# eflynn8/pharmacophore-diffusion

Hardware: AMD Instinct MI355X
Metric: denoising steps/sec (batch x T) at 256-atom pocket, 6 centers (higher is better)
Workload: dtype f32; 1 GPU; BASELINE config 2: 256-atom pocket, 6 centers, T=500 schedule, batch=32 per GPU, dev.yml network; batch_per_gpu=32, n_prot=256, n_pharm=6, T=500, parallelism=graphs sharded over 1 GPU(s), no data-path collective

## Files before the change

include/pfdyn.h:

```cpp
#ifndef PFDYN_H
#define PFDYN_H

#include <stdint.h>

#ifdef __cplusplus
extern "C" {
#endif

#define PF_ABI_VERSION 1

typedef struct pf_handle pf_handle;
typedef void* pf_stream;

typedef enum pf_status {
    PF_OK = 0,
    PF_ERR_ARG = -1,
    PF_ERR_HIP = -2,
    PF_ERR_STATE = -3,
    PF_ERR_WEIGHT = -4,
    PF_ERR_EXCHANGE = -5
} pf_status;

#define PF_NORM_MEAN 0
#define PF_NORM_VALUE 1
// ... 112 lines not shown
                        pf_stream stream);
#define PF_NUM_KERNEL_CLASSES 9
int pf_profile_enable(pf_handle* h, uint32_t kernel_mask);
int pf_profile_read(pf_handle* h, double* total_ms , int64_t* launches , pf_stream stream);
int pf_profile_read_train(pf_handle* h, double* total_ms , int64_t* launches , pf_stream stream);
int pf_debug_work(pf_handle* h, double* flops, double* bytes, int64_t* n_edges , double* executed_flops,
                  int64_t* executed_edges , pf_stream stream);
int pf_debug_counts(pf_handle* h, int64_t* out , pf_stream stream);
int pf_debug_kernel_family(pf_handle* h, int32_t layer, int32_t* rows_per_wave);
int pf_debug_ahead(pf_handle* h, int64_t* out , pf_stream stream);
int pf_debug_pa_check(pf_handle* h, int64_t* violations , pf_stream stream);
int pf_debug_xchg_timeouts(pf_handle* h, int32_t* n);
int pf_debug_xchg_fault(pf_handle* h, int32_t drop_word, int32_t poll_max);
int pf_debug_last_eps(pf_handle* h, float* dev_eps_h , float* dev_eps_x , pf_stream stream);
int pf_debug_l0_hoist(pf_handle* h, int32_t* rows_per_wave);
int pf_debug_chain(pf_handle* h, int32_t kind, int32_t layer, int32_t sub, int32_t n_rows, const float* dev_s_in,
                   const float* dev_v_in, float* dev_s_out, float* dev_v_out, pf_stream stream);

#ifdef __cplusplus
}
#endif
#endif
```

pharmacophore-diffusion_amd/_lib.py:

```python
import ctypes
import os

_HERE = os.path.dirname(os.path.abspath(__file__))
LIB_PATH = os.environ.get("PFDYN_LIB") or os.path.join(_HERE, "csrc", "libpfdyn.so")

PF_ABI_VERSION = 1
PF_NORM_MEAN, PF_NORM_VALUE, PF_NORM_GRAPH = 0, 1, 2


class PfConfig(ctypes.Structure):
    _fields_ = [
        ("abi_version", ctypes.c_int32), ("pharm_nf", ctypes.c_int32), ("rec_nf", ctypes.c_int32),
        ("vector_size", ctypes.c_int32), ("n_hidden_scalars", ctypes.c_int32), ("n_convs", ctypes.c_int32),
        ("n_message_gvps", ctypes.c_int32), ("n_update_gvps", ctypes.c_int32), ("n_noise_gvps", ctypes.c_int32),
        ("message_norm_mode", ctypes.c_int32), ("message_norm_value", ctypes.c_float),
        ("ff_k", ctypes.c_int32), ("pf_k", ctypes.c_int32),
        ("cutoff_pp", ctypes.c_float), ("cutoff_pf", ctypes.c_float), ("cutoff_fp", ctypes.c_float),
        ("cutoff_ff", ctypes.c_float), ("rbf_dmax", ctypes.c_float), ("rbf_dim", ctypes.c_int32),
    ]


class PfStepCoef(ctypes.Structure):
    _fields_ = [("t", ctypes.c_float), ("alpha_t_given_s", ctypes.c_float), ("var_terms", ctypes.c_float),
                ("sigma", ctypes.c_float), ("ep_zt", ctypes.c_float), ("ep_pred", ctypes.c_float)]
# ... 40 lines not shown
    "pf_debug_get_edges": (_I64, [_P, _I32, _P, _P, _I64, _P]),
    "pf_debug_conv_layer": (ctypes.c_int, [_P, _I32] + [_P] * 11),
    "pf_profile_enable": (ctypes.c_int, [_P, ctypes.c_uint32]),
    "pf_profile_read": (ctypes.c_int, [_P, ctypes.POINTER(ctypes.c_double), ctypes.POINTER(_I64), _P]),
    "pf_profile_read_train": (ctypes.c_int, [_P, ctypes.POINTER(ctypes.c_double), ctypes.POINTER(_I64), _P]),
    "pf_debug_work": (ctypes.c_int, [_P, ctypes.POINTER(ctypes.c_double), ctypes.POINTER(ctypes.c_double),
                                     ctypes.POINTER(_I64), ctypes.POINTER(ctypes.c_double), ctypes.POINTER(_I64), _P]),
    "pf_debug_counts": (ctypes.c_int, [_P, ctypes.POINTER(_I64), _P]),
    "pf_debug_kernel_family": (ctypes.c_int, [_P, ctypes.c_int32, ctypes.POINTER(ctypes.c_int32)]),
    "pf_debug_last_eps": (ctypes.c_int, [_P, _P, _P, _P]),
    "pf_debug_xchg_timeouts": (ctypes.c_int, [_P, ctypes.POINTER(ctypes.c_int32)]),
    "pf_debug_xchg_fault": (ctypes.c_int, [_P, _I32, _I32]),
    "pf_debug_ahead": (ctypes.c_int, [_P, ctypes.POINTER(_I64), _P]),
    "pf_debug_pa_check": (ctypes.c_int, [_P, ctypes.POINTER(_I64), _P]),
    "pf_debug_l0_hoist": (ctypes.c_int, [_P, ctypes.POINTER(ctypes.c_int32)]),
    "pf_debug_chain": (ctypes.c_int, [_P, _I32, _I32, _I32, _I32, _P, _P, _P, _P, _P]),
}

_lib = None


def load():
    global _lib
    if _lib is not None:
        return _lib
    if not os.path.exists(LIB_PATH):
        raise ImportError(
            f"{LIB_PATH} is missing: the HIP extension has not been built "
            "(run `python -c 'import __graft_entry__ as g; g.build()'` or `make -C pharmacophore-diffusion_amd/csrc`). "
            "There is no CPU fallback.")
# ... 19 lines not shown
```

pharmacophore-diffusion_amd/csrc/pf_device.h:

```cpp
#pragma once
#include <stdint.h>

#define PF_S 128
#define PF_V 16
#define PF_R 16
#define PF_MAXF 64
#define PF_MAXK 16
#define PF_MAX_GVPS 8

enum { ET_FF = 0, ET_PF = 1, ET_FP = 2, ET_PP = 3 };

#if defined(__HIP_DEVICE_COMPILE__)
#define PF_AS1 __attribute__((address_space(1)))
#else
#define PF_AS1
#endif
typedef const float PF_AS1* pf_gcf;

struct GvpW {
    pf_gcf a_wh;
    pf_gcf a_wu;
    pf_gcf a_main;
    pf_gcf a_main_c;
    pf_gcf a_gate_c;
// ... 123 lines not shown
    const int* ptype;
    const int* eorig;
    const int* l0_gid;
    const float* l0c;
    int ngroups_sel;
    const int* need; int need_stamp;
    int pa_abs;
    pf_gcf n16[4]; int n16_stride[4];
    int uni_base[3], uni_s01, uni_s2g, uni_pa_groups;
    int ptab16_off[4];
    const float* pcen; int pcen_nf;
    const float* x0_static;
    const int* pa_skip;
    int* cnt_snap;
    int* pa_gstamp; int pa_serial;
};

#define L0H_WR 0
#define L0H_WSH 2048
#define L0H_B 4224
#define L0H_WH0 4352
#define L0H_WU 4384
#define L0H_BG 4672
#define L0H_WHT 4736
#define L0H_WHT_PF 21120
#define L0H_B_PF 37504
#define L0H_SIZE (37504 + 128)
#define L0C_WHT_FF 0
#define L0C_B_FF 16384
#define L0C_WHT_FP 16512
#define L0C_B_FP 32896
// ... 253 lines not shown
```

pharmacophore-diffusion_amd/csrc/pf_host.cpp:

```cpp
#include <hip/hip_runtime.h>

#include <algorithm>
#include <cmath>
#include <cstdio>
#include <cstdlib>
#include <cstring>
#include <ctime>
#include <map>
#include <string>
#include <unordered_map>
#include <climits>
#include <vector>

#include "../../include/pfdyn.h"
#include "pf_device.h"
#include "pf_train.h"

#define L0_PTAB_SLOTS 2048

extern "C" {
void pfk_edge_msg(const EdgeParams* p, int layer0, hipStream_t s);
void pfk_edge_msg_coop(const EdgeParams* p, int layer0, hipStream_t s);
void pfk_edge_msg_coop2(const EdgeParams* p, int layer0, hipStream_t s);
void pfk_node_update_coop(const NodeParams* p, int layer0, hipStream_t s);
// ... 80 lines not shown

static void linspace_f32(float start, float end, int steps, float* out) {
    const float step = (end - start) / (float)(steps - 1);
    const int half = steps / 2;
    for (int i = 0; i < steps; ++i) out[i] = i < half ? start + step * (float)i : end - step * (float)(steps - i - 1);
}

}

struct LaunchPolicy {
    static constexpr int kCUs = 256, kSIMDs = 4 * kCUs;
    int n16_mask = 7;
    int tail_graphs_max = 256;
    int xcd_split = 1;
    int edge_rec = 1;
    int node_static = 1;
    int node_xcds = 2;
    int fused_uni = 1;
    int xchg_sleep = 1, hsb_avoid = 0;
    int hs_build = 1;
    int tail_form = 4;
    long n16_fuse_rows_max = 20000;
    long n16_rows_max = 24000;
    int rg_rows_max = 1 << 30;
    int rg2_rows_min = 12000;
    int rg2_rows_min_node = 12000;
    int rg2p_rows_min = 11000;
    int rg2_rows_min_hoist = 30000;
    int l0_rga = 0, l0_rgp = 0;
    int rg_split_max = 128;
// ... 11 lines not shown
        geti("PFDYN_COOP_EDGE_MAX", coop_edge_max); geti("PFDYN_COOP_NODE_MAX", coop_node_max);
        if (const char* e = getenv("PFDYN_COOP2_EDGE_MAX")) coop2_edge_max = coop2_dense_max = atoi(e);
        if (const char* e = getenv("PFDYN_RG_SPLIT_MAX")) rg_split_max = rg_split_max_node = rg_split_max_head = atoi(e);
        geti("PFDYN_RG_SPLIT_MAX_NODE", rg_split_max_node); geti("PFDYN_RG_SPLIT_MAX_HEAD", rg_split_max_head);
        geti("PFDYN_RG_ROWS_MAX", rg_rows_max);
        if (const char* e = getenv("PFDYN_RG2_ROWS_MIN")) rg2_rows_min = rg2_rows_min_hoist = rg2p_rows_min = rg2_rows_min_node = atoi(e);
        geti("PFDYN_RG2P_ROWS_MIN", rg2p_rows_min); geti("PFDYN_RG2_ROWS_MIN_NODE", rg2_rows_min_node); geti("PFDYN_RG2_ROWS_MIN_HOIST", rg2_rows_min_hoist);
        geti("PFDYN_L0_RGP", l0_rgp); geti("PFDYN_L0_RGA", l0_rga);
        for (const char* v : {"PFDYN_RG2_ROWS_MIN", "PFDYN_RG2P_ROWS_MIN", "PFDYN_RG2_ROWS_MIN_HOIST", "PFDYN_RG_SPLIT_MAX", "PFDYN_L0_RGA",
                              "PFDYN_L0_RGP", "PFDYN_RG_ROWS_MAX"})
            if (getenv(v)) n16_mask = 0;
        geti("PFDYN_N16", n16_mask);
        geti("PFDYN_TAIL_GRAPHS_MAX", tail_graphs_max);
        geti("PFDYN_XCD_SPLIT", xcd_split);
        geti("PFDYN_EDGE_REC", edge_rec);
        geti("PFDYN_NODE_XCDS", node_xcds); geti("PFDYN_NODE_STATIC", node_static); geti("PFDYN_HS_BUILD", hs_build); geti("PFDYN_FUSED_UNI", fused_uni); geti("PFDYN_XCHG_SLEEP", xchg_sleep); geti("PFDYN_HSB_AVOID", hsb_avoid);
        if (const char* e = getenv("PFDYN_TAIL_FORM")) tail_form = (e[0] == 'n' || atoi(e) == 16) ? 16 : 4;
        if (const char* e = getenv("PFDYN_N16_ROWS_MAX")) n16_rows_max = n16_fuse_rows_max = atol(e);
        if (const char* e = getenv("PFDYN_N16_FUSE_ROWS_MAX")) n16_fuse_rows_max = atol(e);
    }
};

struct pf_handle {
    LaunchPolicy pol;
    pf_config cfg{};
    bool spec = true, wide = false;
    std::vector<size_t> wide_off;
    WideGvp* d_wgvp = nullptr;
    size_t wide_out_w = 0, wide_out_b = 0;
    std::string err;
// ... 78 lines not shown
    int xchg_fault = 0, xchg_poll_max = 0;
    size_t n16_l0h[4] = {0, 0, 0, 0}, n16_l0h_stride[4] = {0, 0, 0, 0};
    size_t l0c_off = 0;
    bool cen_hoist = true;
    float *d_cen_h = nullptr, *d_cen_p = nullptr, *d_snap[2] = {nullptr, nullptr};
    unsigned int* d_xchg2 = nullptr;
    int snap_cur = -1;
    std::vector<float> t_plan; size_t plan_pos = 0;
    bool cen_valid = false; float cen_t = 0.f; uint64_t cen_wver = 0;
    bool last_cen = false;
    bool pa_spec = true;
    bool spec_valid = false; float spec_t = 0.f; uint64_t spec_wver = 0;
    int step_id = 2;
    int *d_pa_stamp = nullptr, *d_pa_same = nullptr;
    bool e0_saved = false; EdgeParams e0{}; EncodeParams ep0{}; int e0_groups = 0;
    int last_spec = 0;
    int* d_pa_cnt = nullptr;
    int pa_spec_split = 0;
    bool pa_check = false;
    int pa_serial = 0, spec_serial = 0;
    int* d_pa_gstamp = nullptr;
    unsigned long long* d_pa_chk = nullptr;
    bool no_fixed_shapes = false;
    ScaleArgs pend_scale{}; bool has_pend_scale = false;
    bool no_fix_fuse = false;
    bool train_bf16 = false;
    bool train_node_save = true;
    std::vector<float*> t_nsv_z, t_nsv_g, t_nsv_v;
    std::vector<char> t_node_saved;
    std::vector<int> t_grp;
// ... 748 lines not shown
        lp.nt = m; lp.t_dev = nullptr; lp.ptab = h->d_ptab + (size_t)slot0 * slot_floats;
        pfk_l0_hoist(&lp, 1, s);
    }
}

static void n16_refresh(pf_handle* h, hipStream_t s) {
    if (!h->n16_stale) return;
    pfk_gather_weights(h->d_flat, h->d_map + h->n16_begin, h->n_packed - h->n16_begin, h->d_w + h->n16_begin, s);
    if (h->n_split_tab) pfk_n16_split_words(h->d_flat, h->d_split_tab, h->n_split_tab, h->d_w, s);
    h->n16_stale = false;
}

static int run_dynamics_wide(pf_handle* h, float* eps_h, float* eps_x, hipStream_t s, const float* t_scalar) {
    const pf_config& c = h->cfg;
    h->tail_done = false; h->last_tail = 0; h->last_hoist = 0;
    h->cen_valid = false; h->last_cen = false; h->spec_valid = false; h->last_spec = 0; h->e0_saved = false;
    if (h->share_ok && h->share_check == 0) (void)share_now(h);
    if (h->share_check == 2)
        PF_FAIL(h, PF_ERR_ARG, "pf_set_pocket_groups: the claim made for this batch is false -- a graph differs from its representative in "
                               "coordinates or features (compared on the device); bind the batch again without the claim");
    const int S = c.n_hidden_scalars, V = c.vector_size;
    WideEncParams ep{};
    ep.Np = h->Np; ep.Nf = h->Nf; ep.S = S; ep.rec_nf = c.rec_nf; ep.pharm_nf = c.pharm_nf;
    ep.prot_h0 = h->d_prot_h0; ep.pharm_h = h->d_pharm_h;
    ep.t = t_scalar ? nullptr : h->d_t; ep.t_scalar = t_scalar ? *t_scalar : 0.f; ep.gid = h->d_gid;
    for (int nt = 0; nt < 2; ++nt) {
        ep.w[nt] = h->d_w + h->enc_w[nt]; ep.b[nt] = h->d_w + h->enc_b[nt];
        ep.ln_w[nt] = h->d_w + h->enc_lw[nt]; ep.ln_b[nt] = h->d_w + h->enc_lb[nt];
    }
    ep.h_out = h->d_h[0];
    { ProfScope ps(h, pf_handle::K_ENCODE, s); pfk_wide_encode(&ep, s); }
// ... 120 lines not shown
    }
    if (l == 0 && dc.cen_have && h->n16_l0h[ET_FF] != 0) {
        for (int et : {(int)ET_FF, (int)ET_FP}) { e.n16[et] = h->d_w + h->n16_l0h[et]; e.n16_stride[et] = (int)h->n16_l0h_stride[et]; }
        e.pcen = h->d_cen_p; e.pcen_nf = h->Nf; h->last_cen = true;
    }
    e.ngroups_sel = region_groups(h, shared, 0, e.nreg, 16);
    int stride[3], cap[3], grp[3] = {0, 0, 0};
    bool uni = l == 0 && h->pol.fused_uni && !shared && e.reg == h->d_reg && e.nreg == 4 * h->B && h->B <= 64 && !e.pa_abs && !e.need &&
               uniform_regions(h, 3, stride, cap);
    for (int et = 0; et < 3 && uni; ++et) { grp[et] = (cap[et] + 15) / 16; uni = grp[et] > 0 && grp[et] < 8; }
    if (uni) {
        for (int et = 0; et < 3; ++et) e.uni_base[et] = h->h_reg[(size_t)et * h->B];
        e.uni_s01 = stride[0] | (stride[1] << 16);
        e.uni_s2g = stride[2] | (grp[0] << 16) | (grp[1] << 19) | (grp[2] << 22) | ((h->B - 1) << 25);
        e.uni_pa_groups = region_groups(h, shared, 3 * h->B, 4 * h->B, 16);
    }
    dc.rg = 4;
    if (l == 0 && e.x0_static && pa_ahead_ok(h, e, shared)) {
        e.cnt_snap = h->d_pa_cnt;
        h->e0 = e; h->ep0 = dc.ep; h->e0_saved = true;
        h->e0_groups = region_groups(h, shared, 3 * h->B, 4 * h->B, 16);
    }
}
static void edge_launch(DynCall& dc, int l) {
    pf_handle* h = dc.h; hipStream_t s = dc.s; const pf_config& c = h->cfg; const bool train = dc.train;
    const bool last = dc.last = (l == c.n_convs - 1), pruned = dc.pruned = (l == prune_layer(h));
    EdgeParams& e = dc.e; int &rg = dc.rg, &rgp = dc.rgp;
    e = edge_params_base(h, l, last, pruned);
    e.h = train ? h->t_H[l] : h->d_h[dc.cur]; e.v = train ? h->t_V[l] : h->d_v[dc.cur];
    e.msg_s = train ? h->t_msg_s[l] : h->d_msg_s; e.msg_v = train ? h->t_msg_v[l] : h->d_msg_v;
    if (dc.fuse_l0node && l == 1) { e.msg_s = h->d_msg_s2; e.msg_v = h->d_msg_v2; }
    e.pre = (l == 0 && dc.pre_ready) ? h->d_pre : nullptr;
    if (train) { e.sv_z = h->t_sv_z[l]; e.sv_g = h->t_sv_g[l]; e.sv_v = h->t_sv_v[l]; e.sv_stride = (size_t)std::max<int64_t>(h->Ecap, 1); }
    const bool shared = dc.shared = dc.share && pruned && l == 0;
    if ((last || pruned) && h->rg_compact && (last ? 2 : 4) * h->B <= 1024) {
        e.reg = shared ? h->d_reg_share : h->d_reg; e.regB = h->B; e.nreg = (last ? 2 : 4) * h->B; e.pa_abs = shared ? 1 : 0;
        if (shared) { e.need = h->d_need; e.need_stamp = h->edges_stamp; }
        e.ngroups4 = region_groups(h, shared, 0, e.nreg, 4); e.ngroups8 = region_groups(h, shared, 0, e.nreg, 8);
    }
    if (train && h->train_bf16) e.bf16 = 1;
    rg = train ? ((h->train_rg_edge && h->train_rg_node && !h->train_bf16) ? h->pol.rg_mode(e.ntiles) : 0)
               : h->pol.rg_mode(shared ? (int)((h->share_rows + 31) / 32) : e.ntiles);
    rgp = 0;
// ... 87 lines not shown
    pf_handle* h = dc.h; const StepParams* step = dc.step;
    cp.on = 1; cp.Nf = h->Nf; cp.nf = h->cfg.pharm_nf; cp.t_next = t_next; cp.pharm_h = h->d_snap[h->snap_cur]; cp.noise = step->noise;
    cp.a_ts = step->a_ts; cp.var = step->var; cp.sigma = step->sigma; cp.ep_zt = step->ep_zt; cp.ep_pred = step->ep_pred; cp.ep_feat = step->ep_feat;
    cp.enc_w = h->d_w + h->enc_w[1]; cp.enc_b = h->d_w + h->enc_b[1]; cp.enc_lw = h->d_w + h->enc_lw[1]; cp.enc_lb = h->d_w + h->enc_lb[1];
    cp.blk = h->d_w + h->l0c_off; cp.cen_h = h->d_cen_h; cp.cen_p = h->d_cen_p; cp.xchg2 = hp.xchg2 = h->d_xchg2;
    h->cen_valid = true; h->cen_t = t_next; h->cen_wver = h->w_version;
}
static int pa_ahead_plan(DynCall& dc, EdgeParams& es, EncodeParams& ees) {
    pf_handle* h = dc.h; const pf_config& c = h->cfg;
    if (!(h->e0_saved && h->pa_spec && !h->t_plan.empty() && dc.t_scalar && h->d_pa_stamp && !share_next(h))) return 0;
    float tn = planned_next_t(h, *dc.t_scalar, nullptr);
    if (tn != tn) return 0;
    l0_prepare_t(h, &tn, 1, dc.s);
    uint32_t bits; memcpy(&bits, &tn, 4);
    es = h->e0; es.pa_skip = nullptr; es.pcen = nullptr;
    es.ptab = h->d_ptab + (size_t)h->ptab_slot[bits] * L0_NTAB * c.rec_nf * PF_S;
    for (int et = 0; et < 4; ++et) { es.n16[et] = h->d_w + h->n16_l0[et]; es.n16_stride[et] = (int)h->n16_l0_stride[et]; }
    ees = h->ep0; ees.t_scalar = tn;
    h->spec_valid = true; h->spec_t = tn; h->spec_wver = h->w_version;
    es.pa_serial = h->spec_serial = ++h->pa_serial; es.pa_gstamp = h->d_pa_gstamp;
    return h->e0_groups;
}
static void merged_step_launch(DynCall& dc, const NodeParams& n, HeadParams& hp) {
    pf_handle* h = dc.h; hipStream_t s = dc.s; const pf_config& c = h->cfg;
    hp.xchg = h->d_xchg; hp.xchg_fault = h->xchg_fault;
    CenHoistParams cp{}; EdgeParams es{}; EncodeParams ees{};
    const float t_next = cen_hoist_plan(dc);
    const int spec_groups = pa_ahead_plan(dc, es, ees);
    if (t_next == t_next) cen_hoist_params(dc, t_next, cp, hp);
    const bool sn = share_next(h);
// ... 68 lines not shown
        up.sv_z = h->t_hsv_z; up.sv_g = h->t_hsv_g; up.sv_v = h->t_hsv_v; up.sv_stride = (size_t)h->Nf;
        { ProfScope ps(h, pf_handle::K_HEAD, s); pfk_rg_unit(&up, s); }
        h->t_head_saved = true; dc.head_done = true;
    }
    if (!dc.head_done) { ProfScope ps(h, pf_handle::K_HEAD, s); if (hp.ntiles <= h->pol.coop_node_max) pfk_noise_head_coop(&hp, s); else pfk_noise_head(&hp, s); }
}
static int run_dynamics(pf_handle* h, float* eps_h, float* eps_x, hipStream_t s, const float* t_scalar = nullptr, bool train = false, const StepParams* step = nullptr) {
    if (h->wide && !train) return run_dynamics_wide(h, eps_h, eps_x, s, t_scalar);
    const pf_config& c = h->cfg;
    h->tail_done = false; h->last_tail = 0;
    DynCall dc{};
    dc.h = h; dc.s = s; dc.eps_h = eps_h; dc.eps_x = eps_x; dc.t_scalar = t_scalar; dc.train = train; dc.step = step;
    dc.cen_have = !train && h->cen_valid && h->edges_built && t_scalar != nullptr && *t_scalar == h->cen_t && h->cen_wver == h->w_version;
    h->cen_valid = false; h->last_cen = false;
    dc.spec_have = !train && h->spec_valid && h->edges_built && t_scalar != nullptr && *t_scalar == h->spec_t && h->spec_wver == h->w_version;
    h->spec_valid = false; h->last_spec = 0; h->e0_saved = false;
    if (!train) n16_refresh(h, s);
    dc.ep = encode_params(h, t_scalar, train ? h->t_H[0] : h->d_h[0]);
    if (const int rc = dyn_prologue(dc)) return rc;
    dyn_hoist_prepare(dc);
    h->last_hoist = 0;
    dc.fuse_l0node = !train && dc.n16_batch && (long)h->n_edge_tiles_act * 32 <= h->pol.n16_fuse_rows_max && (h->pol.n16_mask & 4) && (h->pol.n16_mask & 1) && dc.hoist && c.n_convs == 2 && prune_layer(h) == 0 && c.pf_k > 0 &&
                     c.n_update_gvps >= 1 && h->rg_compact && 2 * h->B <= 1024 && h->d_msg_s2 != nullptr && h->n16_fused[0] != 0;
    for (int l = 0; l < c.n_convs; ++l, dc.cur ^= 1) { edge_launch(dc, l); node_launch(dc, l); }
    head_launch(dc);
    h->edges_built = h->tail_done;
    hipError_t e = hipGetLastError();
    if (e != hipSuccess) PF_FAIL(h, PF_ERR_HIP, "kernel launch failed: %s", hipGetErrorString(e));
    return PF_OK;
}

// ... 1931 lines not shown
    else if (kind == 1) {
        if (sub > 1) PF_FAIL(h, PF_ERR_ARG, "pf_debug_chain: node type 0 (prot) or 1 (pharm)");
        p.stream = h->d_w + h->rg_upd[(size_t)layer * 2 + sub]; p.n_gvps = c.n_update_gvps;
    } else if (kind == 2) {
        const size_t* lo = &h->ln_off[(size_t)(layer * 2 + (sub >> 1)) * 4];
        p.ln_w = h->d_w + lo[(sub & 1) * 2]; p.ln_b = h->d_w + lo[(sub & 1) * 2 + 1];
    } else {
        p.stream = h->d_w + h->rg_upd[(size_t)(c.n_convs - 1) * 2 + 1]; p.n_gvps = c.n_noise_gvps; p.skip_gvps = c.n_update_gvps;
    }
    pfk_rg_unit(&p, (hipStream_t)stream);
    hipError_t e = hipGetLastError();
    if (e != hipSuccess) PF_FAIL(h, PF_ERR_HIP, "kernel launch failed: %s", hipGetErrorString(e));
    return PF_OK;
}

int pf_debug_l0_hoist(pf_handle* h, int32_t* rows_per_wave) {
    if (!h || !rows_per_wave) return PF_ERR_ARG;
    *rows_per_wave = h->last_hoist;
    return PF_OK;
}

int pf_profile_enable(pf_handle* h, uint32_t kernel_mask) {
    if (!h) return PF_ERR_ARG;
    h->prof_mask = kernel_mask;
    return PF_OK;
}

static int profile_read_range(pf_handle* h, int k0, int k1, double* total_ms, int64_t* launches, pf_stream stream) {
    if (!h || !total_ms || !launches) return PF_ERR_ARG;
    PF_HIP(h, hipStreamSynchronize((hipStream_t)stream));
// ... 84 lines not shown
```

pharmacophore-diffusion_amd/csrc/pf_n16.hip:

```cpp
#include <hip/hip_runtime.h>
#include <type_traits>
#include <algorithm>
#include "pf_device.h"
#ifdef N16_STAMPS
#define N16_STAMP_GLOBALS 1
namespace {
__device__ unsigned long long* g_n16_stamps = nullptr;
__device__ int g_n16_stamp_off = 0;
__device__ int g_n16_stamp_kid = -1;
}
#define SB_STAMP(k)                                                                                                    \
    do {                                                                                                               \
        const int rb_ = (int)blockIdx.x - g_n16_stamp_off;                                                             \
        if ((k) < 16 && (threadIdx.x & 63) == 0 && g_n16_stamps && rb_ >= 0 && rb_ < 64 && (g_n16_stamp_kid < 0 || g_n16_stamp_kid == 3)) \
            g_n16_stamps[((size_t)rb_ * 4 + (threadIdx.x >> 6)) * 64 + 40 + (k)] = __builtin_amdgcn_s_memtime();       \
    } while (0)
#endif
#include "pf_stepbuild.h"

#include "pf_n16_core.h"

using namespace pfn16;

namespace {
// ... 141 lines not shown
    const int rs = a_reg[r];
    const int ng = ((c + 15) >> 4) - keep;
    int incl = ng;
    incl += dpp_i<0x111>(incl); incl += dpp_i<0x112>(incl); incl += dpp_i<0x114>(incl); incl += dpp_i<0x118>(incl);
    incl += dpp_ir<0x142, 0xa>(incl); incl += dpp_ir<0x143, 0xc>(incl);
    const unsigned long long m = __ballot(incl > w);
    if (!m) return;
    const int l = __builtin_amdgcn_readfirstlane(__ffsll((long long)m) - 1);
    const int first = __builtin_amdgcn_readlane(incl - ng, l);
    const int cnt = __builtin_amdgcn_readlane(c, l), start = __builtin_amdgcn_readlane(rs, l);
    const int loc = (w - first + __builtin_amdgcn_readlane(keep, l)) << 4;
    const int e0 = start + loc;
    const int nv = __builtin_amdgcn_readfirstlane(min(16, cnt - loc));
    const int e = e0 + min(j, nv - 1);
    n16_edge_item<N16_M0H>(p, ep, &lds, e, a_esrc[e], a_edst[e], nv, (int)ET_PP, lane, wq, sk);
}

struct N16LnPre { float a, b; };
__device__ __forceinline__ N16LnPre n16_ln_request(pf_gcf w1, pf_gcf b1, pf_gcf w2, pf_gcf b2, const int lane, const int wq) {
    const int t = wq * 64 + lane;
    N16LnPre q;
    q.a = (t < 128 ? w1 : b1)[t & 127];
    q.b = (t < 128 ? w2 : b2)[t & 127];
    return q;
}
__device__ __forceinline__ void n16_ln_stage(const N16LnPre& q, N16Lds* lds, const int lane, const int wq) {
    const int t = wq * 64 + lane;
    lds->ln[t] = q.a;
    lds->ln[256 + t] = q.b;
}
// ... 590 lines not shown
        }
    }
}

}

extern "C" {
void pfk_n16_edge(const EdgeParams* p, const EncodeParams* enc, int layer0, hipStream_t s) {
    if (p->ntiles == 0) return;
    const int grid = p->nreg > 0 ? p->ngroups_sel : p->ntiles * 2;
    if (grid <= 0) return;
    const EncodeParams noenc{};
    if (layer0 && p->uni_s2g != 0) {
        const int B = p->regB;
        const int nstat = B * (((p->uni_s2g >> 16) & 7) + ((p->uni_s2g >> 19) & 7) + ((p->uni_s2g >> 22) & 7));
        hipLaunchKernelGGL(k_n16_edge_u, dim3(nstat + p->uni_pa_groups), dim3(256), 0, s, p->dyn_cnt, p->esrc, p->edst, p->uni_base[0],
                           p->uni_base[1], p->uni_base[2], p->uni_s01, p->uni_s2g, p->reg, *p, *enc);
        return;
    }
    if (layer0) hipLaunchKernelGGL((k_n16_edge<true>), dim3(grid), dim3(256), 0, s, p->dyn_cnt, p->reg, p->nreg, p->regB, p->pa_abs, *p, *enc);
    else hipLaunchKernelGGL((k_n16_edge<false>), dim3(grid), dim3(256), 0, s, p->dyn_cnt, p->reg, p->nreg, p->regB, p->pa_abs, *p, noenc);
}
#ifdef N16_STAMPS
int pfk_n16_set_stamp_buffer(unsigned long long* dev, int off) {
    (void)hipMemcpyToSymbol(HIP_SYMBOL(g_n16_stamp_off), &off, sizeof(off));
    return (int)hipMemcpyToSymbol(HIP_SYMBOL(g_n16_stamps), &dev, sizeof(dev));
}
int pfk_n16_set_stamp_kernel(int kid) { return (int)hipMemcpyToSymbol(HIP_SYMBOL(g_n16_stamp_kid), &kid, sizeof(kid)); }
#endif
#ifdef N16_TRACE
int pfk_n16_set_trace_buffer(unsigned long long* dev) { return (int)hipMemcpyToSymbol(HIP_SYMBOL(g_n16_trace), &dev, sizeof(dev)); }
// ... 25 lines not shown
```

pharmacophore-diffusion_amd/csrc/pf_n16_core.h:

```cpp
#pragma once
#include <hip/hip_runtime.h>
#include <type_traits>
#include <algorithm>
#include "pf_device.h"

typedef float f32x4 __attribute__((ext_vector_type(4)));

namespace pfn16 {

template <int I, int N, class F>
__device__ __forceinline__ void static_for(F&& f) {
    if constexpr (I < N) {
        f(std::integral_constant<int, I>{});
        static_for<I + 1, N>(f);
    }
}

__device__ __forceinline__ float rcpf_(float x) { return __builtin_amdgcn_rcpf(x); }
__device__ __forceinline__ float sqrtf_(float x) { return __builtin_amdgcn_sqrtf(x); }
__device__ __forceinline__ float rsqf_(float x) { return __builtin_amdgcn_rsqf(x); }
__device__ __forceinline__ float sigmoidf_(float x) { return rcpf_(1.0f + __expf(-x)); }
__device__ __forceinline__ float siluf_(float x) { return x * rcpf_(1.0f + __expf(-x)); }

__device__ __forceinline__ f32x4 mfma16(const float a, const float b, const f32x4 c) {
// ... 466 lines not shown
        for (int r = 0; r < 4; ++r) S[t][r] = seg_scan16(S[t][r], sm);
#pragma unroll
    for (int r = 0; r < 4; ++r) VB[r] = seg_scan16(VB[r], sm);
    if (tail) {
        float* ms = p.msg_s + (size_t)rw.e * PF_S + 32 * wq + 4 * g;
        *reinterpret_cast<f32x4*>(ms) = S[0];
        *reinterpret_cast<f32x4*>(ms + 16) = S[1];
        if (wq < 3) {
            float* mv = p.msg_v + (size_t)rw.e * 48 + 12 * g + wq;
#pragma unroll
            for (int r = 0; r < 4; ++r) mv[3 * r] = VB[r];
        }
    }
}

template <int KIND0>
__device__ __forceinline__ void n16_edge_item(const EdgeParams& p, const EncodeParams& ep, N16Lds* lds, const int e, const int src,
                                              const int dst, const int nv, const int et, const int lane, const int wq, int& sk) {
    N16_STAMP(sk, lane, wq);
    N16Ring ring;
    ring_start(ring, p.n16[et] + (size_t)wq * p.n16_stride[et], lane);
    const int g = lane >> 4;
    N16Rows rw;
    rw.e = e;
    rw.dst = dst;
    if (et == ET_PP && p.x0_static) {
        const float* a = p.x0_static + (size_t)src * 3;
        const float* b = p.x0_static + (size_t)rw.dst * 3;
        rw.xs = make_float4(a[0], a[1], a[2], 0.f); rw.xd = make_float4(b[0], b[1], b[2], 0.f);
    } else { rw.xs = p.xn[src]; rw.xd = p.xn[rw.dst]; }
    float XS[32], VB[4];
    f32x4 S[2];
    S[0] = (f32x4){0.f, 0.f, 0.f, 0.f}; S[1] = S[0];
    if constexpr (KIND0 == N16_M0H) {
        pf_gcf tp;
        if (et == ET_PP || et == ET_PF) {
            int ty = p.ptype[src] * PF_S + p.ptab16_off[et];
            if (p.ptab_gstride) ty += p.l0_gid[src] * p.ptab_gstride;
            tp = (pf_gcf)p.ptab + ty;
        } else tp = (pf_gcf)p.pcen + ((size_t)(et == ET_FP ? p.pcen_nf : 0) + (size_t)(src - ep.Np)) * PF_S;
        tp += 32 * wq + 4 * g;
        S[0] = *reinterpret_cast<const f32x4 PF_AS1*>(tp);
        S[1] = *reinterpret_cast<const f32x4 PF_AS1*>(tp + 16);
    }
    if constexpr (KIND0 == N16_M0Z) {
        const float tt = ep.t ? ((pf_gcf)ep.t)[((const int PF_AS1*)ep.gid)[src]] : ep.t_scalar;
        n16_encode_pharm(ep, (pf_gcf)ep.pharm_h + (size_t)(src - ep.Np) * ep.pharm_nf, tt, XS, lds, lane, wq);
    }
    if constexpr (KIND0 == N16_M0F) {
        const f32x4 PF_AS1* hp = reinterpret_cast<const f32x4 PF_AS1*>((pf_gcf)p.h + (size_t)src * PF_S) + g;
#pragma unroll
        for (int T = 0; T < 8; ++T) {
            const f32x4 x = hp[4 * T];
#pragma unroll
            for (int r = 0; r < 4; ++r) XS[4 * T + r] = x[r];
        }
        pf_gcf vp = (pf_gcf)p.v + (size_t)src * 48 + 12 * g + (wq < 3 ? wq : 0);
#pragma unroll
// ... 11 lines not shown
```

pharmacophore-diffusion_amd/csrc/pf_stepbuild.h:

```cpp
#pragma once
#include <hip/hip_runtime.h>
#include "pf_device.h"

#ifndef SB_STAMP
#define SB_STAMP(k)
#endif
#ifdef SB_CUT
#define SB_PHASE(k) do { SB_STAMP(k); if ((k) == SB_CUT) __builtin_amdgcn_endpgm(); } while (0)
#else
#define SB_PHASE(k) SB_STAMP(k)
#endif

namespace pfsb {

constexpr int SB_MAXA = 512;
constexpr int SB_MAXNF = 16;

__device__ __forceinline__ float sqdist_rn(const float4 a, const float4 b) {
#pragma clang fp contract(off)
    const float dx = a.x - b.x, dy = a.y - b.y, dz = a.z - b.z;
    const float xx = dx * dx, yy = dy * dy, zz = dz * dz;
    return (xx + yy) + zz;
}
__device__ __forceinline__ unsigned long long dkey(const float d2, const int idx) {
// ... 575 lines not shown
        const bool pa_on = p.act_ids && !p.pa_static;
        const int n_pa16 = pa_on ? 16 * (int)((all >> 16) & 0xfffu) : 0;
        auto fp_store = [&](const int t, const int pr, const unsigned int r0, const unsigned int r1, const int e0) {
            const int pc = pr & 0xffff, fl = pr >> 16;
            const int below = fl < 32 ? __popc(r0 & ((1u << fl) - 1u)) : __popc(r0) + __popc(r1 & ((1u << (fl - 32)) - 1u));
            p.esrc[e0 + below] = GF + fl;
            p.edst[e0 + below] = p0 + pc;
            if (p.rec) {
                const float4 xs = L.px[pc], xd = L.fx[fl];
                const int2 pa = L.a_pa[pc];
                const int ty = (int)L.a_ty[pc];
                int4* r = p.rec + (size_t)3 * (reg_pf + t);
                r[0] = make_int4(__builtin_bit_cast(int, xs.x), __builtin_bit_cast(int, xs.y), __builtin_bit_cast(int, xs.z), (p0 + pc) | (ty << 24));
                r[1] = make_int4(__builtin_bit_cast(int, xd.x), __builtin_bit_cast(int, xd.y), __builtin_bit_cast(int, xd.z), GF + fl);
                r[2] = make_int4(e0, __popc(r0) + __popc(r1), pa.x, pa.y);
            }
        };
        auto pa_store = [&](const int4 a4, const int k, const int src) {
            const int c = a4.x, e0 = reg_pa + a4.y, dg = a4.z, ps = a4.w;
            if (k < dg) {
                p.esrc[e0 + k] = src;
                p.edst[e0 + k] = p0 + c;
                if (p.eorig) p.eorig[e0 + k] = ps + k;
            }
            if (k == 15)
                for (int k2 = 16; k2 < dg; ++k2) {
                    p.esrc[e0 + k2] = p.esrc[ps + k2];
                    p.edst[e0 + k2] = p0 + c;
                    if (p.eorig) p.eorig[e0 + k2] = ps + k2;
                }
// ... 135 lines not shown
```

pharmacophore-diffusion_amd/engine.py:

```python
import ctypes
from typing import Dict, Optional

import torch

from . import _lib as L


def _stream_ptr():
    return ctypes.c_void_p(torch.cuda.current_stream().cuda_stream)


def _dptr(t: Optional[torch.Tensor]):
    if t is None:
        return None
    assert t.is_cuda and t.is_contiguous(), "device tensors must be contiguous CUDA/HIP tensors"
    return ctypes.c_void_p(t.data_ptr())


def _i32_host(t: torch.Tensor):
    import numpy as np
    a = t.detach().cpu().numpy() if isinstance(t, torch.Tensor) else np.asarray(t)
    return np.ascontiguousarray(a, dtype=np.int32)


# ... 359 lines not shown

    def pa_check_counts(self):
        out = (ctypes.c_int64 * 3)()
        with torch.cuda.device(self.device):
            self._ck(self.lib.pf_debug_pa_check(self._h, out, _stream_ptr()), "pf_debug_pa_check")
        return dict(zip(("violations", "checked", "exposed"), list(out)))

    def pa_check(self) -> int:
        return self.pa_check_counts()["violations"]

    def l0_hoist(self) -> int:
        r = ctypes.c_int32()
        self._ck(self.lib.pf_debug_l0_hoist(self._h, ctypes.byref(r)), "pf_debug_l0_hoist")
        return int(r.value)

    def debug_chain(self, kind: int, layer: int, sub: int, s_in: torch.Tensor, v_in: torch.Tensor):
        s_in = s_in.to(self.device, torch.float32).contiguous()
        v_in = v_in.to(self.device, torch.float32).contiguous()
        n = s_in.shape[0]
        if kind == 3:
            s_out = torch.empty(n, self.cfg.pharm_nf, device=self.device)
            v_out = torch.empty(n, 3, device=self.device)
        else:
            s_out = torch.empty(n, 128, device=self.device)
            v_out = torch.empty(n, 16, 3, device=self.device)
        with torch.cuda.device(self.device):
            self._ck(self.lib.pf_debug_chain(self._h, int(kind), int(layer), int(sub), int(n), _dptr(s_in), _dptr(v_in),
                                             _dptr(s_out), _dptr(v_out), _stream_ptr()), "pf_debug_chain")
        return s_out, v_out

# ... 22 lines not shown
```

Measured before the change: 686,200 sample-steps/s.

## Feed layer-0 edge kernel from packed edge records and LDS-staged type table

Adds a new layer-0 uniform edge kernel that reads source/destination coordinates, type and indices from the packed per-edge records written at edge-build time, broadcast across lanes with ds_bpermute. It also stages the small per-type table into LDS per wave, replacing scattered global gathers through esrc/edst, ptype and x0. The step builder now writes an extra reversed record for PF edges. The intent is to cut dependent gather latency in the first message layer. The cost is extra record writes, more LDS use, and a path that only applies when rec_nf is at most 16 and the table is not strided per group.

```diff
diff --git a/include/pfdyn.h b/include/pfdyn.h
--- a/include/pfdyn.h
+++ b/include/pfdyn.h
@@ -150,6 +150,7 @@
 int pf_debug_xchg_fault(pf_handle* h, int32_t drop_word, int32_t poll_max);
 int pf_debug_last_eps(pf_handle* h, float* dev_eps_h , float* dev_eps_x , pf_stream stream);
 int pf_debug_l0_hoist(pf_handle* h, int32_t* rows_per_wave);
+int pf_debug_l0_rec(pf_handle* h, int32_t* on);
 int pf_debug_chain(pf_handle* h, int32_t kind, int32_t layer, int32_t sub, int32_t n_rows, const float* dev_s_in,
                    const float* dev_v_in, float* dev_s_out, float* dev_v_out, pf_stream stream);
 
diff --git a/pharmacophore-diffusion_amd/_lib.py b/pharmacophore-diffusion_amd/_lib.py
--- a/pharmacophore-diffusion_amd/_lib.py
+++ b/pharmacophore-diffusion_amd/_lib.py
@@ -78,6 +78,7 @@
     "pf_debug_ahead": (ctypes.c_int, [_P, ctypes.POINTER(_I64), _P]),
     "pf_debug_pa_check": (ctypes.c_int, [_P, ctypes.POINTER(_I64), _P]),
     "pf_debug_l0_hoist": (ctypes.c_int, [_P, ctypes.POINTER(ctypes.c_int32)]),
+    "pf_debug_l0_rec": (ctypes.c_int, [_P, ctypes.POINTER(ctypes.c_int32)]),
     "pf_debug_chain": (ctypes.c_int, [_P, _I32, _I32, _I32, _I32, _P, _P, _P, _P, _P]),
 }
 
diff --git a/pharmacophore-diffusion_amd/csrc/pf_device.h b/pharmacophore-diffusion_amd/csrc/pf_device.h
--- a/pharmacophore-diffusion_amd/csrc/pf_device.h
+++ b/pharmacophore-diffusion_amd/csrc/pf_device.h
@@ -161,7 +161,9 @@
     const int* pa_skip;
     int* cnt_snap;
     int* pa_gstamp; int pa_serial;
-};
+    const int4* rec; int tab_rows;
+};
+#define L0_TAB_ROWS 16
 
 #define L0H_WR 0
 #define L0H_WSH 2048
diff --git a/pharmacophore-diffusion_amd/csrc/pf_host.cpp b/pharmacophore-diffusion_amd/csrc/pf_host.cpp
--- a/pharmacophore-diffusion_amd/csrc/pf_host.cpp
+++ b/pharmacophore-diffusion_amd/csrc/pf_host.cpp
@@ -118,6 +118,7 @@
     int tail_graphs_max = 256;
     int xcd_split = 1;
     int edge_rec = 1;
+    int l0_rec = 1;
     int node_static = 1;
     int node_xcds = 2;
     int fused_uni = 1;
@@ -159,6 +160,7 @@
         geti("PFDYN_TAIL_GRAPHS_MAX", tail_graphs_max);
         geti("PFDYN_XCD_SPLIT", xcd_split);
         geti("PFDYN_EDGE_REC", edge_rec);
+        geti("PFDYN_L0_REC", l0_rec);
         geti("PFDYN_NODE_XCDS", node_xcds); geti("PFDYN_NODE_STATIC", node_static); geti("PFDYN_HS_BUILD", hs_build); geti("PFDYN_FUSED_UNI", fused_uni); geti("PFDYN_XCHG_SLEEP", xchg_sleep); geti("PFDYN_HSB_AVOID", hsb_avoid);
         if (const char* e = getenv("PFDYN_TAIL_FORM")) tail_form = (e[0] == 'n' || atoi(e) == 16) ? 16 : 4;
         if (const char* e = getenv("PFDYN_N16_ROWS_MAX")) n16_rows_max = n16_fuse_rows_max = atol(e);
@@ -267,6 +269,7 @@
     int step_id = 2;
     int *d_pa_stamp = nullptr, *d_pa_same = nullptr;
     bool e0_saved = false; EdgeParams e0{}; EncodeParams ep0{}; int e0_groups = 0;
+    int last_l0rec = 0;
     int last_spec = 0;
     int* d_pa_cnt = nullptr;
     int pa_spec_split = 0;
@@ -1045,7 +1048,7 @@
 static int run_dynamics_wide(pf_handle* h, float* eps_h, float* eps_x, hipStream_t s, const float* t_scalar) {
     const pf_config& c = h->cfg;
     h->tail_done = false; h->last_tail = 0; h->last_hoist = 0;
-    h->cen_valid = false; h->last_cen = false; h->spec_valid = false; h->last_spec = 0; h->e0_saved = false;
+    h->cen_valid = false; h->last_cen = false; h->spec_valid = false; h->last_spec = 0; h->last_l0rec = 0; h->e0_saved = false;
     if (h->share_ok && h->share_check == 0) (void)share_now(h);
     if (h->share_check == 2)
         PF_FAIL(h, PF_ERR_ARG, "pf_set_pocket_groups: the claim made for this batch is false -- a graph differs from its representative in "
@@ -1196,7 +1199,11 @@
         e.uni_s01 = stride[0] | (stride[1] << 16);
         e.uni_s2g = stride[2] | (grp[0] << 16) | (grp[1] << 19) | (grp[2] << 22) | ((h->B - 1) << 25);
         e.uni_pa_groups = region_groups(h, shared, 3 * h->B, 4 * h->B, 16);
-    }
+        if (h->pol.l0_rec && h->rec_valid && h->d_rec && e.ptab && e.ptab_gstride == 0 && c.rec_nf <= L0_TAB_ROWS) {
+            e.rec = h->d_rec; e.tab_rows = c.rec_nf;
+        }
+    }
+    if (l == 0) h->last_l0rec = e.rec != nullptr ? 1 : 0;
     dc.rg = 4;
     if (l == 0 && e.x0_static && pa_ahead_ok(h, e, shared)) {
         e.cnt_snap = h->d_pa_cnt;
@@ -1209,6 +1216,7 @@
     const bool last = dc.last = (l == c.n_convs - 1), pruned = dc.pruned = (l == prune_layer(h));
     EdgeParams& e = dc.e; int &rg = dc.rg, &rgp = dc.rgp;
     e = edge_params_base(h, l, last, pruned);
+    if (l == 0) h->last_l0rec = 0;
     e.h = train ? h->t_H[l] : h->d_h[dc.cur]; e.v = train ? h->t_V[l] : h->d_v[dc.cur];
     e.msg_s = train ? h->t_msg_s[l] : h->d_msg_s; e.msg_v = train ? h->t_msg_v[l] : h->d_msg_v;
     if (dc.fuse_l0node && l == 1) { e.msg_s = h->d_msg_s2; e.msg_v = h->d_msg_v2; }
@@ -1326,6 +1334,7 @@
     l0_prepare_t(h, &tn, 1, dc.s);
     uint32_t bits; memcpy(&bits, &tn, 4);
     es = h->e0; es.pa_skip = nullptr; es.pcen = nullptr;
+    es.rec = nullptr; es.tab_rows = 0;
     es.ptab = h->d_ptab + (size_t)h->ptab_slot[bits] * L0_NTAB * c.rec_nf * PF_S;
     for (int et = 0; et < 4; ++et) { es.n16[et] = h->d_w + h->n16_l0[et]; es.n16_stride[et] = (int)h->n16_l0_stride[et]; }
     ees = h->ep0; ees.t_scalar = tn;
@@ -1424,7 +1433,7 @@
     dc.cen_have = !train && h->cen_valid && h->edges_built && t_scalar != nullptr && *t_scalar == h->cen_t && h->cen_wver == h->w_version;
     h->cen_valid = false; h->last_cen = false;
     dc.spec_have = !train && h->spec_valid && h->edges_built && t_scalar != nullptr && *t_scalar == h->spec_t && h->spec_wver == h->w_version;
-    h->spec_valid = false; h->last_spec = 0; h->e0_saved = false;
+    h->spec_valid = false; h->last_spec = 0; h->last_l0rec = 0; h->e0_saved = false;
     if (!train) n16_refresh(h, s);
     dc.ep = encode_params(h, t_scalar, train ? h->t_H[0] : h->d_h[0]);
     if (const int rc = dyn_prologue(dc)) return rc;
@@ -3386,6 +3395,12 @@
     return PF_OK;
 }
 
+int pf_debug_l0_rec(pf_handle* h, int32_t* on) {
+    if (!h || !on) return PF_ERR_ARG;
+    *on = h->last_l0rec;
+    return PF_OK;
+}
+
 int pf_debug_l0_hoist(pf_handle* h, int32_t* rows_per_wave) {
     if (!h || !rows_per_wave) return PF_ERR_ARG;
     *rows_per_wave = h->last_hoist;
diff --git a/pharmacophore-diffusion_amd/csrc/pf_n16.hip b/pharmacophore-diffusion_amd/csrc/pf_n16.hip
--- a/pharmacophore-diffusion_amd/csrc/pf_n16.hip
+++ b/pharmacophore-diffusion_amd/csrc/pf_n16.hip
@@ -179,6 +179,93 @@
     const int nv = __builtin_amdgcn_readfirstlane(min(16, cnt - loc));
     const int e = e0 + min(j, nv - 1);
     n16_edge_item<N16_M0H>(p, ep, &lds, e, a_esrc[e], a_edst[e], nv, (int)ET_PP, lane, wq, sk);
+}
+
+__global__ __launch_bounds__(256) void k_n16_edge_ur(const int* __restrict__ a_dyn_cnt, const int4* __restrict__ a_rec, const int a_b0,
+                                                     const int a_b1, const int a_b2, const int a_s01, const int a_s2g,
+                                                     const int* __restrict__ a_reg, const EdgeParams p, const EncodeParams ep) {
+    __shared__ N16Lds lds;
+    __shared__ __attribute__((aligned(16))) float ltab[4 * L0_TAB_ROWS * 32];
+    const int lane = threadIdx.x & 63;
+    const int wq = __builtin_amdgcn_readfirstlane((int)(threadIdx.x >> 6));
+    const int j = lane & 15;
+    int sk = 0;
+    N16_STAMP(sk, lane, wq);
+#ifdef N16_STAMPS
+    struct WgTimes { __device__ ~WgTimes() { if (on) g_n16_stamps[(size_t)blockIdx.x * 2 + 1] = __builtin_amdgcn_s_memrealtime(); } bool on; } wgt_;
+    wgt_.on = g_n16_stamp_kid == 100 && g_n16_stamps && threadIdx.x == 0 && blockIdx.x < 8192;
+    if (wgt_.on) g_n16_stamps[(size_t)blockIdx.x * 2] = __builtin_amdgcn_s_memrealtime();
+#endif
+    const int gff = (a_s2g >> 16) & 7, gpf = (a_s2g >> 19) & 7, gfp = (a_s2g >> 22) & 7, a_B = (int)((unsigned)a_s2g >> 25) + 1;
+    const int nff = a_B * gff, npf = a_B * gpf, nfp = a_B * gfp;
+    int w = (int)blockIdx.x;
+    if (p.cnt_snap && w == 0 && threadIdx.x < 64 && lane < a_B) p.cnt_snap[lane] = a_dyn_cnt[3 * a_B + lane];
+    float* const tabw = ltab + wq * (L0_TAB_ROWS * 32);
+    f32x4 tq[2];
+    auto tab_request = [&](const int et) {
+        pf_gcf tb = (pf_gcf)p.ptab + p.ptab16_off[et] + 32 * wq + 4 * (lane & 7);
+#pragma unroll
+        for (int i = 0; i < 2; ++i) tq[i] = *reinterpret_cast<const f32x4 PF_AS1*>(tb + min(8 * i + (lane >> 3), p.tab_rows - 1) * PF_S);
+    };
+    auto tab_park = [&]() {
+#pragma unroll
+        for (int i = 0; i < 2; ++i) *reinterpret_cast<f32x4*>(tabw + 4 * (64 * i + lane)) = tq[i];
+        __builtin_amdgcn_wave_barrier();
+    };
+    if (w < nff + npf + nfp) {
+        int et, base, stride, gk;
+        if (w < nff) { et = ET_FF; base = a_b0; stride = a_s01 & 0xffff; gk = gff; }
+        else if (w < nff + npf) { w -= nff; et = ET_PF; base = a_b1; stride = (int)((unsigned)a_s01 >> 16); gk = gpf; }
+        else { w -= nff + npf; et = ET_FP; base = a_b2; stride = a_s2g & 0xffff; gk = gfp; }
+        const int g = w / gk, k = w - g * gk;
+        const int e0 = base + g * stride + 16 * k;
+        const int cnt = a_dyn_cnt[et * a_B + g];
+        const int4* rp = a_rec + (size_t)3 * (e0 + j);
+        const int4 r0 = rp[0], r1 = rp[1];
+        if (et == ET_PF) tab_request(et);
+        const int nv = __builtin_amdgcn_readfirstlane(min(16, cnt - 16 * k));
+        if (nv <= 0) return;
+        const int jj = min(j, nv - 1);
+        const int from = 4 * ((lane & 48) | jj);
+        const int sw = __builtin_amdgcn_ds_bpermute(from, r0.w), dst = __builtin_amdgcn_ds_bpermute(from, r1.w);
+        N16Rec rc;
+        rc.xs = make_float4(__builtin_bit_cast(float, __builtin_amdgcn_ds_bpermute(from, r0.x)),
+                            __builtin_bit_cast(float, __builtin_amdgcn_ds_bpermute(from, r0.y)),
+                            __builtin_bit_cast(float, __builtin_amdgcn_ds_bpermute(from, r0.z)), 0.f);
+        rc.xd = make_float4(__builtin_bit_cast(float, __builtin_amdgcn_ds_bpermute(from, r1.x)),
+                            __builtin_bit_cast(float, __builtin_amdgcn_ds_bpermute(from, r1.y)),
+                            __builtin_bit_cast(float, __builtin_amdgcn_ds_bpermute(from, r1.z)), 0.f);
+        rc.ty = (int)((unsigned)sw >> 24);
+        const int src = sw & 0xffffff;
+        if (et == ET_PF) {
+            tab_park();
+            n16_edge_item<N16_M0H>(p, ep, &lds, e0 + jj, src, dst, nv, et, lane, wq, sk, &rc, tabw);
+        } else if (p.pcen) n16_edge_item<N16_M0H>(p, ep, &lds, e0 + jj, src, dst, nv, et, lane, wq, sk, &rc);
+        else n16_edge_item<N16_M0Z>(p, ep, &lds, e0 + jj, src, dst, nv, et, lane, wq, sk, &rc);
+        return;
+    }
+    w -= nff + npf + nfp;
+    const int r = 3 * a_B + min(lane, a_B - 1);
+    const int c = lane < a_B ? a_dyn_cnt[r] : 0;
+    const int keep = p.pa_skip ? min(p.pa_skip[min(lane, a_B - 1)], (c + 15) >> 4) : 0;
+    const int rs = a_reg[r];
+    tab_request((int)ET_PP);
+    const int ng = ((c + 15) >> 4) - keep;
+    int incl = ng;
+    incl += dpp_i<0x111>(incl); incl += dpp_i<0x112>(incl); incl += dpp_i<0x114>(incl); incl += dpp_i<0x118>(incl);
+    incl += dpp_ir<0x142, 0xa>(incl); incl += dpp_ir<0x143, 0xc>(incl);
+    const unsigned long long m = __ballot(incl > w);
+    if (!m) return;
+    const int l = __builtin_amdgcn_readfirstlane(__ffsll((long long)m) - 1);
+    const int first = __builtin_amdgcn_readlane(incl - ng, l);
+    const int cnt = __builtin_amdgcn_readlane(c, l), start = __builtin_amdgcn_readlane(rs, l);
+    const int loc = (w - first + __builtin_amdgcn_readlane(keep, l)) << 4;
+    const int e0 = start + loc;
+    const int nv = __builtin_amdgcn_readfirstlane(min(16, cnt - loc));
+    const int e = e0 + min(j, nv - 1);
+    const int src = p.esrc[e], dst = p.edst[e];
+    tab_park();
+    n16_edge_item<N16_M0H>(p, ep, &lds, e, src, dst, nv, (int)ET_PP, lane, wq, sk, nullptr, tabw);
 }
 
 struct N16LnPre { float a, b; };
@@ -799,7 +886,10 @@
     if (layer0 && p->uni_s2g != 0) {
         const int B = p->regB;
         const int nstat = B * (((p->uni_s2g >> 16) & 7) + ((p->uni_s2g >> 19) & 7) + ((p->uni_s2g >> 22) & 7));
-        hipLaunchKernelGGL(k_n16_edge_u, dim3(nstat + p->uni_pa_groups), dim3(256), 0, s, p->dyn_cnt, p->esrc, p->edst, p->uni_base[0],
+        if (p->rec && p->tab_rows > 0 && p->tab_rows <= L0_TAB_ROWS)
+            hipLaunchKernelGGL(k_n16_edge_ur, dim3(nstat + p->uni_pa_groups), dim3(256), 0, s, p->dyn_cnt, p->rec, p->uni_base[0], p->uni_base[1],
+                               p->uni_base[2], p->uni_s01, p->uni_s2g, p->reg, *p, *enc);
+        else hipLaunchKernelGGL(k_n16_edge_u, dim3(nstat + p->uni_pa_groups), dim3(256), 0, s, p->dyn_cnt, p->esrc, p->edst, p->uni_base[0],
                            p->uni_base[1], p->uni_base[2], p->uni_s01, p->uni_s2g, p->reg, *p, *enc);
         return;
     }
diff --git a/pharmacophore-diffusion_amd/csrc/pf_n16_core.h b/pharmacophore-diffusion_amd/csrc/pf_n16_core.h
--- a/pharmacophore-diffusion_amd/csrc/pf_n16_core.h
+++ b/pharmacophore-diffusion_amd/csrc/pf_n16_core.h
@@ -504,9 +504,14 @@
     }
 }
 
+struct N16Rec {
+    float4 xs, xd;
+    int ty;
+};
 template <int KIND0>
 __device__ __forceinline__ void n16_edge_item(const EdgeParams& p, const EncodeParams& ep, N16Lds* lds, const int e, const int src,
-                                              const int dst, const int nv, const int et, const int lane, const int wq, int& sk) {
+                                              const int dst, const int nv, const int et, const int lane, const int wq, int& sk,
+                                              const N16Rec* rc = nullptr, const float* ltab = nullptr) {
     N16_STAMP(sk, lane, wq);
     N16Ring ring;
     ring_start(ring, p.n16[et] + (size_t)wq * p.n16_stride[et], lane);
@@ -514,7 +519,8 @@
     N16Rows rw;
     rw.e = e;
     rw.dst = dst;
-    if (et == ET_PP && p.x0_static) {
+    if (rc) { rw.xs = rc->xs; rw.xd = rc->xd; }
+    else if (et == ET_PP && p.x0_static) {
         const float* a = p.x0_static + (size_t)src * 3;
         const float* b = p.x0_static + (size_t)rw.dst * 3;
         rw.xs = make_float4(a[0], a[1], a[2], 0.f); rw.xd = make_float4(b[0], b[1], b[2], 0.f);
@@ -523,15 +529,21 @@
     f32x4 S[2];
     S[0] = (f32x4){0.f, 0.f, 0.f, 0.f}; S[1] = S[0];
     if constexpr (KIND0 == N16_M0H) {
-        pf_gcf tp;
-        if (et == ET_PP || et == ET_PF) {
-            int ty = p.ptype[src] * PF_S + p.ptab16_off[et];
-            if (p.ptab_gstride) ty += p.l0_gid[src] * p.ptab_gstride;
-            tp = (pf_gcf)p.ptab + ty;
-        } else tp = (pf_gcf)p.pcen + ((size_t)(et == ET_FP ? p.pcen_nf : 0) + (size_t)(src - ep.Np)) * PF_S;
-        tp += 32 * wq + 4 * g;
-        S[0] = *reinterpret_cast<const f32x4 PF_AS1*>(tp);
-        S[1] = *reinterpret_cast<const f32x4 PF_AS1*>(tp + 16);
+        if (ltab && (et == ET_PP || et == ET_PF)) {
+            const float* tl = ltab + min(rc ? rc->ty : p.ptype[src], L0_TAB_ROWS - 1) * 32 + 4 * g;
+            S[0] = *reinterpret_cast<const f32x4*>(tl);
+            S[1] = *reinterpret_cast<const f32x4*>(tl + 16);
+        } else {
+            pf_gcf tp;
+            if (et == ET_PP || et == ET_PF) {
+                int ty = (rc ? rc->ty : p.ptype[src]) * PF_S + p.ptab16_off[et];
+                if (p.ptab_gstride) ty += p.l0_gid[src] * p.ptab_gstride;
+                tp = (pf_gcf)p.ptab + ty;
+            } else tp = (pf_gcf)p.pcen + ((size_t)(et == ET_FP ? p.pcen_nf : 0) + (size_t)(src - ep.Np)) * PF_S;
+            tp += 32 * wq + 4 * g;
+            S[0] = *reinterpret_cast<const f32x4 PF_AS1*>(tp);
+            S[1] = *reinterpret_cast<const f32x4 PF_AS1*>(tp + 16);
+        }
     }
     if constexpr (KIND0 == N16_M0Z) {
         const float tt = ep.t ? ((pf_gcf)ep.t)[((const int PF_AS1*)ep.gid)[src]] : ep.t_scalar;
diff --git a/pharmacophore-diffusion_amd/csrc/pf_stepbuild.h b/pharmacophore-diffusion_amd/csrc/pf_stepbuild.h
--- a/pharmacophore-diffusion_amd/csrc/pf_stepbuild.h
+++ b/pharmacophore-diffusion_amd/csrc/pf_stepbuild.h
@@ -613,6 +613,9 @@
                 r[0] = make_int4(__builtin_bit_cast(int, xs.x), __builtin_bit_cast(int, xs.y), __builtin_bit_cast(int, xs.z), (p0 + pc) | (ty << 24));
                 r[1] = make_int4(__builtin_bit_cast(int, xd.x), __builtin_bit_cast(int, xd.y), __builtin_bit_cast(int, xd.z), GF + fl);
                 r[2] = make_int4(e0, __popc(r0) + __popc(r1), pa.x, pa.y);
+                int4* rf = p.rec + (size_t)3 * (e0 + below);
+                rf[0] = make_int4(__builtin_bit_cast(int, xd.x), __builtin_bit_cast(int, xd.y), __builtin_bit_cast(int, xd.z), GF + fl);
+                rf[1] = make_int4(__builtin_bit_cast(int, xs.x), __builtin_bit_cast(int, xs.y), __builtin_bit_cast(int, xs.z), p0 + pc);
             }
         };
         auto pa_store = [&](const int4 a4, const int k, const int src) {
diff --git a/pharmacophore-diffusion_amd/engine.py b/pharmacophore-diffusion_amd/engine.py
--- a/pharmacophore-diffusion_amd/engine.py
+++ b/pharmacophore-diffusion_amd/engine.py
@@ -397,6 +397,11 @@
         self._ck(self.lib.pf_debug_l0_hoist(self._h, ctypes.byref(r)), "pf_debug_l0_hoist")
         return int(r.value)
 
+    def l0_rec(self) -> bool:
+        r = ctypes.c_int32()
+        self._ck(self.lib.pf_debug_l0_rec(self._h, ctypes.byref(r)), "pf_debug_l0_rec")
+        return bool(r.value)
+
     def debug_chain(self, kind: int, layer: int, sub: int, s_in: torch.Tensor, v_in: torch.Tensor):
         s_in = s_in.to(self.device, torch.float32).contiguous()
         v_in = v_in.to(self.device, torch.float32).contiguous()
```

After: 696,200 sample-steps/s, median of 6. 1.01x the previous value.
